# CZY-Code/PHNet

Hardware: AMD Instinct MI355X
Metric: clips/s (5x3x320x800) fwd+bwd (higher is better)
Workload: dtype f32 storage / accumulation, every product as an EXACT three-term bf16 split (6 bf16 MFMAs, f32-MFMA accuracy); 1 GPU; 5-frame clip 3x320x800, resnet34 + router + lane head, fwd+bwd+AdamW, 1 clip/GPU/step, random-init weights; parallelism=dp1, launch=hipGraph replay of the whole step

## Files before the change

### phnet_amd/csrc/assign.hip

```cpp
#include "assign_device.h"

namespace {

using namespace phassign;

__global__ __launch_bounds__(4 * NT) void lane_assign_kernel(
    const float* __restrict__ pred, const float* __restrict__ tgt, int N, int L, int S, float img_w, float img_h,
    int64_t* __restrict__ rows_by_col, int64_t* __restrict__ rows_sorted, int32_t* __restrict__ n_valid_out,
    float* __restrict__ cost_out)
{
    extern __shared__ float cost[];
    lane_assign_block<false, 4>(pred, tgt, N, L, S, img_w, img_h, rows_by_col, rows_sorted, n_valid_out, cost_out, cost);
}

__global__ __launch_bounds__(4 * NT) void lane_assign_tokens_kernel(
    const float* __restrict__ pred, const float* __restrict__ tgt, int N, int L, int S, float img_w, float img_h,
    int64_t* __restrict__ rows_by_col, int64_t* __restrict__ rows_sorted, const float* __restrict__ feat, int E,
    float* __restrict__ tokens, unsigned char* __restrict__ valid)
{
    extern __shared__ float cost[];
    float* part = cost + N * MAXL;
    const int e = threadIdx.x % E, grp = threadIdx.x / E, groups = (4 * NT) / E;
    float s = 0.f;
    if (grp < groups)
        for (int n = grp; n < N; n += groups) s += feat[(size_t)n * E + e];
    lane_assign_block<false, 4>(pred, tgt, N, L, S, img_w, img_h, rows_by_col, rows_sorted, nullptr, nullptr, cost);
    if (grp < groups) part[grp * E + e] = s;
    __syncthreads();
    if (grp != 0) return;
    float total = 0.f;
    for (int g2 = 0; g2 < groups; ++g2) total += part[g2 * E + e];
    float possum = 0.f;
    int cnt = 0;
    for (int l = 0; l < L; ++l) {
        const long long r = rows_sorted[l];
        const bool ok = r >= 0 && r < N;
        const float v = ok ? feat[(size_t)r * E + e] : 0.f;
        tokens[(size_t)l * E + e] = v;
        possum += v;
        cnt += ok;
        if (e == 0) valid[l] = ok;
    }
    tokens[(size_t)L * E + e] = (total - possum) / (float)(N - cnt);
    if (e == 0) valid[L] = 1;
}

__global__ __launch_bounds__(4 * NT) void lane_assign_many_kernel(
    const float* __restrict__ pred, const float* __restrict__ tgt, int N, int L, int S, float img_w, float img_h,
    int64_t* __restrict__ rows, int64_t* __restrict__ cols, int32_t* __restrict__ n_pairs)
{
    extern __shared__ float cost[];
    lane_assign_block<true, 4>(pred, tgt, N, L, S, img_w, img_h, nullptr, nullptr, nullptr, nullptr, cost, 0.5f, rows, cols, n_pairs);
}

}
PHNET_API int phnet_lane_assign(const float* pred, const float* tgt, int32_t N, int32_t L, int32_t S,
                                float img_w, float img_h, int64_t* rows_by_col, int64_t* rows_sorted,
                                int32_t* n_valid, float* cost, void* stream)
{
    if (N < 1 || N > NT || L < 0 || L > MAXL || S < 1 || S > 250) return PHNET_ERR_ARG;
    if (L == 0) return PHNET_OK;
    if (!pred || !tgt || !rows_by_col || !rows_sorted) return PHNET_ERR_ARG;
    hipLaunchKernelGGL(lane_assign_kernel, dim3(1), dim3(4 * NT), (size_t)N * MAXL * sizeof(float), (hipStream_t)stream,
                       pred, tgt, N, L, S, img_w, img_h, rows_by_col, rows_sorted, n_valid, cost);
    return phnet_launch_status();
}

PHNET_API int phnet_lane_assign_one2many(const float* pred, const float* tgt, int32_t N, int32_t L, int32_t S,
                                         float img_w, float img_h, int64_t* rows, int64_t* cols, int32_t* n_pairs, void* stream)
{
    if (N < 1 || N > NT || L < 1 || L > MAXL || S < 1 || S > 250) return PHNET_ERR_ARG;
    if (!pred || !tgt || !rows || !cols) return PHNET_ERR_ARG;
    hipLaunchKernelGGL(lane_assign_many_kernel, dim3(1), dim3(4 * NT), (size_t)2 * N * MAXL * sizeof(float), (hipStream_t)stream,
                       pred, tgt, N, L, S, img_w, img_h, rows, cols, n_pairs);
    return phnet_launch_status();
}

PHNET_API int phnet_lane_assign_tokens(const float* pred, const float* tgt, int32_t N, int32_t L, int32_t S, float img_w, float img_h,
                                       int64_t* rows_by_col, int64_t* rows_sorted, const float* feat, int32_t E,
                                       float* tokens, uint8_t* valid, void* stream)
{
    if (N < 1 || N > NT || L < 1 || L > MAXL || S < 1 || S > 250 || E < 1 || E > 256 || (4 * NT) % E) return PHNET_ERR_ARG;
    if (!pred || !tgt || !rows_by_col || !rows_sorted || !feat || !tokens || !valid) return PHNET_ERR_ARG;
    const size_t lds = ((size_t)N * MAXL + (size_t)4 * NT) * sizeof(float);
    hipLaunchKernelGGL(lane_assign_tokens_kernel, dim3(1), dim3(4 * NT), lds, (hipStream_t)stream,
                       pred, tgt, N, L, S, img_w, img_h, rows_by_col, rows_sorted, feat, E, tokens, valid);
    return phnet_launch_status();
}
```

### phnet_amd/csrc/assign_device.h

```cpp
#pragma once
#include "common.h"

namespace phassign {

constexpr int NT = 256;
constexpr int MAXL = 4;

template <int WAVES = 4>
__device__ __forceinline__ float block_max(float v, float* red) {
    v = wave_max(v);
    __syncthreads();
    if ((threadIdx.x & 63) == 0) red[threadIdx.x >> 6] = v;
    __syncthreads();
    float m = red[0];
#pragma unroll
    for (int i = 1; i < WAVES; ++i) m = fmaxf(m, red[i]);
    return m;
}

template <bool MANY = false, int QUAD = 1>
__device__ __forceinline__ void lane_assign_block(
    const float* __restrict__ pred, const float* __restrict__ tgt, int N, int L, int S, float img_w, float img_h,
    int64_t* __restrict__ rows_by_col, int64_t* __restrict__ rows_sorted, int32_t* __restrict__ n_valid_out,
    float* __restrict__ cost_out, float* cost ,
    float focal_alpha = 0.25f, int64_t* __restrict__ many_rows = nullptr, int64_t* __restrict__ many_cols = nullptr,
    int32_t* __restrict__ many_n = nullptr)
{
    __shared__ float t_x[MAXL][256];
    __shared__ float t_len[MAXL], red[4 * QUAD];
    __shared__ int t_valid[MAXL], top_rows[MAXL][MAXL], best_combo;
    __shared__ float combo_cost[NT];
    __shared__ unsigned char gone[NT];
    __shared__ int ks[MAXL], comp[MAXL], many_count, more;
    const int tid = threadIdx.x;
    const int W = 6 + S;
    if (tid < NT) gone[tid] = 0;

    if (tid < MAXL) {
        t_valid[tid] = (tid < L) && (tgt[tid * W + 1] == 1.0f);
        t_len[tid] = 0.f;
    }
    for (int i = tid; i < L * S; i += NT * QUAD) t_x[i / S][i % S] = tgt[(i / S) * W + 6 + (i % S)];
    __syncthreads();
    if (tid < L) {
        int n = 0;
        for (int k = 0; k < S; ++k) { const float t = t_x[tid][k]; n += !((t < 0.f) || (t >= img_w)); }
        t_len[tid] = (float)n;
    }
    __syncthreads();

    if constexpr (QUAD == 4) {
        const int a = tid & (NT - 1), jq = tid / NT;
        const bool arow = a < N, on = arow && jq < L && t_valid[jq];
        const float* p = pred + (size_t)(arow ? a : 0) * W;
        float cls = 0.f, dist = 0.f, start = 0.f, theta = 0.f, iou = 0.f;
        float mx_d = -INFINITY, mx_s = -INFINITY, mx_t = -INFINITY;
        if (arow) {
            const float pr = 1.0f / (1.0f + expf(-p[1]));
            const float negc = -logf(1.0f - pr + 1e-12f) * (1.0f - focal_alpha) * (pr * pr);
            const float posc = -logf(pr + 1e-12f) * focal_alpha * ((1.0f - pr) * (1.0f - pr));
            cls = posc - negc;
        }
        if (on) {
            float d = 0.f, ovr = 0.f, uni = 0.f;
            const float* tx = t_x[jq];
            auto term = [&](int k, float xr) {
                const float x = xr * (img_w - 1.0f), t = tx[k];
                const bool ok = !(t < 0.f) && !(t >= img_w);
                d += ok ? fabsf(t - x) : 0.f;
                ovr += ok ? fminf(x + 15.f, t + 15.f) - fmaxf(x - 15.f, t - 15.f) : 0.f;
                uni += ok ? fmaxf(x + 15.f, t + 15.f) - fminf(x - 15.f, t - 15.f) : 0.f;
            };
            int k = 0;
            if ((W & 1) == 0) {
                for (; k + 1 < S; k += 16) {
                    float2 buf[8];
#pragma unroll
                    for (int u = 0; u < 8; ++u) {
                        const int kk = k + 2 * u;
                        buf[u] = *reinterpret_cast<const float2*>(p + 6 + (kk + 1 < S ? kk : 0));
                    }
#pragma unroll
                    for (int u = 0; u < 8; ++u) {
                        const int kk = k + 2 * u;
                        if (kk + 1 < S) { term(kk, buf[u].x); term(kk + 1, buf[u].y); }
                    }
                }
                k = S & ~1;
            }
            for (; k < S; ++k) term(k, p[6 + k]);
            dist = d / (t_len[jq] + 1e-9f);
            iou = ovr / (uni + 1e-9f);
            const float* tr = tgt + (size_t)jq * W;
            const float dy = p[2] * (img_h - 1.0f) - tr[2] * (img_h - 1.0f), dx = p[3] * (img_w - 1.0f) - tr[3] * (img_w - 1.0f);
            start = sqrtf(dy * dy + dx * dx);
            theta = fabsf(p[4] - tr[4]) * 180.f;
            mx_d = dist; mx_s = start; mx_t = theta;
        }
        mx_d = block_max<16>(mx_d, red);
        mx_s = block_max<16>(mx_s, red);
        mx_t = block_max<16>(mx_t, red);
        if (arow) {
            float c = INFINITY;
            if (on) {
                const float a_ = 1.0f - dist / (mx_d + 1e-4f);
                const float b_ = 1.0f - start / (mx_s + 1e-4f);
                const float t_ = 1.0f - theta / (mx_t + 1e-4f);
                const float prod = a_ * b_ * t_;
                c = -(prod * prod) * 3.0f + cls - iou;
            }
            cost[a * MAXL + jq] = c;
            if (MANY) cost[(N + a) * MAXL + jq] = on ? fmaxf(iou, 0.f) : -1.f;
            if (cost_out && jq < L) cost_out[(size_t)a * L + jq] = c;
        }
    } else {
    float dist[MAXL], start[MAXL], theta[MAXL], iou[MAXL], cls = 0.f;
    float mx_d = -INFINITY, mx_s = -INFINITY, mx_t = -INFINITY;
    const bool arow = tid < N;
    if (arow) {
        const float* p = pred + (size_t)tid * W;
        const float pr = 1.0f / (1.0f + expf(-p[1]));
        const float negc = -logf(1.0f - pr + 1e-12f) * (1.0f - focal_alpha) * (pr * pr);
        const float posc = -logf(pr + 1e-12f) * focal_alpha * ((1.0f - pr) * (1.0f - pr));
        cls = posc - negc;
        const float psy = p[2] * (img_h - 1.0f), psx = p[3] * (img_w - 1.0f), pth = p[4];
        float d[MAXL], ovr[MAXL], uni[MAXL];
#pragma unroll
        for (int j = 0; j < MAXL; ++j) d[j] = ovr[j] = uni[j] = 0.f;
        bool col_on[MAXL];
#pragma unroll
        for (int j = 0; j < MAXL; ++j) col_on[j] = j < L && t_valid[j];
        auto term = [&](int k, float xr) {
            const float x = xr * (img_w - 1.0f);
#pragma unroll
            for (int j = 0; j < MAXL; ++j) {
                const float t = t_x[j][k];
                const bool ok = col_on[j] && !(t < 0.f) && !(t >= img_w);
                d[j] += ok ? fabsf(t - x) : 0.f;
                ovr[j] += ok ? fminf(x + 15.f, t + 15.f) - fmaxf(x - 15.f, t - 15.f) : 0.f;
                uni[j] += ok ? fmaxf(x + 15.f, t + 15.f) - fminf(x - 15.f, t - 15.f) : 0.f;
            }
        };
        int k = 0;
        if ((W & 1) == 0)
            for (; k + 1 < S; k += 16) {
                float2 buf[8];
#pragma unroll
                for (int u = 0; u < 8; ++u) {
                    const int kk = k + 2 * u;
                    buf[u] = *reinterpret_cast<const float2*>(p + 6 + (kk + 1 < S ? kk : 0));
                }
#pragma unroll
                for (int u = 0; u < 8; ++u) {
                    const int kk = k + 2 * u;
                    if (kk + 1 < S) { term(kk, buf[u].x); term(kk + 1, buf[u].y); }
                }
            }
        k = ((W & 1) == 0) ? (S & ~1) : 0;
        for (; k < S; ++k) term(k, p[6 + k]);
#pragma unroll
        for (int j = 0; j < MAXL; ++j) {
            dist[j] = start[j] = theta[j] = iou[j] = 0.f;
            if (j >= L || !t_valid[j]) continue;
            dist[j] = d[j] / (t_len[j] + 1e-9f);
            iou[j] = ovr[j] / (uni[j] + 1e-9f);
            const float* tr = tgt + (size_t)j * W;
            const float dy = psy - tr[2] * (img_h - 1.0f), dx = psx - tr[3] * (img_w - 1.0f);
            start[j] = sqrtf(dy * dy + dx * dx);
            theta[j] = fabsf(pth - tr[4]) * 180.f;
            mx_d = fmaxf(mx_d, dist[j]); mx_s = fmaxf(mx_s, start[j]); mx_t = fmaxf(mx_t, theta[j]);
        }
    }
    mx_d = block_max(mx_d, red);
    mx_s = block_max(mx_s, red);
    mx_t = block_max(mx_t, red);
    if (arow) {
#pragma unroll
        for (int j = 0; j < MAXL; ++j) {
            float c = INFINITY;
            if (j < L && t_valid[j]) {
                const float a = 1.0f - dist[j] / (mx_d + 1e-4f);
                const float b = 1.0f - start[j] / (mx_s + 1e-4f);
                const float t = 1.0f - theta[j] / (mx_t + 1e-4f);
                const float prod = a * b * t;
                c = -(prod * prod) * 3.0f + cls - iou[j];
            }
            cost[tid * MAXL + j] = c;
            if (MANY) cost[(N + tid) * MAXL + j] = (j < L && t_valid[j]) ? fmaxf(iou[j], 0.f) : -1.f;
            if (cost_out && j < L) cost_out[(size_t)tid * L + j] = c;
        }
    }
    }
    __syncthreads();

    if (MANY) {
        const int j = tid >> 6, lane = tid & 63;
        if (j < MAXL) {
            const bool valid = j < L && t_valid[j];
            float sum = 0.f;
            int taken[MAXL];
            for (int r = 0; r < MAXL; ++r) {
                float bv = -INFINITY; int bi = 0x7fffffff;
                if (valid)
                    for (int i = lane; i < N; i += 64) {
                        bool tk = false;
                        for (int q = 0; q < r; ++q) tk |= (taken[q] == i);
                        const float v = cost[(N + i) * MAXL + j];
                        if (!tk && (v > bv || (v == bv && i < bi))) { bv = v; bi = i; }
                    }
#pragma unroll
                for (int off = 32; off > 0; off >>= 1) {
                    const float ov = __shfl_xor(bv, off, 64);
                    const int oi = __shfl_xor(bi, off, 64);
                    if (ov > bv || (ov == bv && oi < bi)) { bv = ov; bi = oi; }
                }
                taken[r] = bi;
                if (valid && bi != 0x7fffffff) sum += bv;
            }
            if (lane == 0) {
                const int k = (int)sum;
                ks[j] = valid ? (k < 1 ? 1 : k) : 0;
            }
        }
        if (tid == 0) many_count = 0;
        __syncthreads();
        if (tid == 0) {
            int c = 0;
            for (int j = 0; j < MAXL; ++j) { comp[j] = c; c += (j < L && t_valid[j]); }
            int kc[MAXL] = {0, 0, 0, 0};
            for (int j = 0; j < MAXL; ++j) if (j < L && t_valid[j]) kc[comp[j]] = ks[j];
            for (int j = 0; j < MAXL; ++j) ks[j] = kc[j];
            more = (kc[0] + kc[1] + kc[2] + kc[3]) > 0;
        }
        __syncthreads();
    }
    for (int round = 0; round < (MANY ? MAXL + 1 : 1); ++round) {
    if (MANY && !more) break;
    {
        const int j = tid >> 6, lane = tid & 63;
        if (j < MAXL) {
            const bool valid = j < L && t_valid[j];
            for (int r = 0; r < MAXL; ++r) {
                float bv = INFINITY; int bi = 0x7fffffff;
                if (valid)
                    for (int i = lane; i < N; i += 64) {
                        bool taken = gone[i] != 0;
                        for (int q = 0; q < r; ++q) taken |= (top_rows[j][q] == i);
                        const float c = cost[i * MAXL + j];
                        if (!taken && (c < bv || (c == bv && i < bi))) { bv = c; bi = i; }
                    }
#pragma unroll
                for (int off = 32; off > 0; off >>= 1) {
                    const float ov = __shfl_xor(bv, off, 64);
                    const int oi = __shfl_xor(bi, off, 64);
                    if (ov < bv || (ov == bv && oi < bi)) { bv = ov; bi = oi; }
                }
                if (lane == 0) top_rows[j][r] = valid ? bi : -1;
                __builtin_amdgcn_wave_barrier();
            }
        }
    }
    __syncthreads();

    {
        int rows[MAXL];
        float total = 0.f;
        bool ok = true;
#pragma unroll
        for (int j = 0; j < MAXL; ++j) {
            const int pick = (tid >> (2 * j)) & 3;
            const bool valid = j < L && t_valid[j];
            rows[j] = valid ? top_rows[j][pick] : -1;
            if (!valid) { ok = ok && pick == 0; continue; }
            if (rows[j] < 0 || rows[j] == 0x7fffffff) { ok = false; continue; }
            total += cost[rows[j] * MAXL + j];
#pragma unroll
            for (int q = 0; q < j; ++q) ok = ok && !(rows[q] >= 0 && rows[q] == rows[j]);
        }
        if (tid < NT) combo_cost[tid] = ok ? total : INFINITY;
    }
    __syncthreads();
    if (tid < 64) {
        float bv = INFINITY; int bi = 0x7fffffff;
        for (int c = tid; c < NT; c += 64) {
            const float v = combo_cost[c];
            if (v < bv || (v == bv && c < bi)) { bv = v; bi = c; }
        }
#pragma unroll
        for (int off = 32; off > 0; off >>= 1) {
            const float ov = __shfl_xor(bv, off, 64);
            const int oi = __shfl_xor(bi, off, 64);
            if (ov < bv || (ov == bv && oi < bi)) { bv = ov; bi = oi; }
        }
        if (tid == 0) best_combo = bi;
    }
    __syncthreads();
    if (tid == 0) {
        int rows[MAXL], nv = 0;
        for (int j = 0; j < MAXL; ++j) {
            const bool valid = j < L && t_valid[j];
            rows[j] = (valid && best_combo != 0x7fffffff) ? top_rows[j][(best_combo >> (2 * j)) & 3] : -1;
            if (j < L && rows_by_col) rows_by_col[j] = rows[j];
            nv += rows[j] >= 0;
        }
        for (int a = 0; a < MAXL; ++a)
            for (int b = a + 1; b < MAXL; ++b) {
                const bool swap = (rows[b] >= 0) && (rows[a] < 0 || rows[b] < rows[a]);
                if (swap) { const int t = rows[a]; rows[a] = rows[b]; rows[b] = t; }
            }
        if (!MANY) {
            for (int j = 0; j < L; ++j) rows_sorted[j] = rows[j];
            if (n_valid_out) *n_valid_out = nv;
        } else {
            int lab[MAXL];
            for (int p_ = 0; p_ < MAXL; ++p_) {
                lab[p_] = -1;
                if (rows[p_] < 0) continue;
                for (int j = 0; j < MAXL; ++j)
                    if (j < L && t_valid[j] && best_combo != 0x7fffffff && top_rows[j][(best_combo >> (2 * j)) & 3] == rows[p_]) lab[p_] = j;
            }
            for (int p_ = 0; p_ < MAXL; ++p_) {
                if (rows[p_] < 0 || ks[p_] <= 0) continue;
                many_rows[many_count] = rows[p_];
                many_cols[many_count] = lab[p_];
                ++many_count;
                gone[rows[p_]] = 1;
            }
            int any = 0;
            for (int j = 0; j < MAXL; ++j) { if (ks[j] > 0) --ks[j]; any += ks[j]; }
            more = any > 0 && nv > 0;
        }
    }
    __syncthreads();
    }
    if (MANY && tid == 0) {
        for (int i = many_count; i < MAXL * MAXL; ++i) { many_rows[i] = -1; many_cols[i] = -1; }
        if (many_n) *many_n = many_count;
    }
}


}
```

### phnet_amd/libs/models/Router4OL.py

```python
import copy
import math

import torch
import torch.nn as nn

from phnet_amd import functional as PF
from phnet_amd.arena import SinkPool, grad_sink
from phnet_amd.trunk import encoder_forward
from ..ops import nms
from ..utils.lane import Lane
from .fpn import FPN
from .resnet import ResNetWrapper
from .Router import AdaptiveRouter4Lane
from .utils.dynamic_head import DynamicConv
from .utils.transformer import TransformerDecoder, TransformerDecoderLayer


def LinearModule(hidden_dim):
    return nn.ModuleList([nn.Linear(hidden_dim, hidden_dim), nn.ReLU(inplace=False)])


class PositionalEncodingLearned(nn.Module):
    def __init__(self, num_embeddings, num_pos_feats=256):
        super().__init__()
# ... 193 lines not shown
        if self.training:
            self.priors, self.priors_on_featmap = self.generate_priors_from_embeddings()
        parts = {k: v.split(1, dim=0) for k, v in self.stage0_front(fmaps0).items()}
        return [{k: parts[k][t] for k in parts} for t in range(fmaps0.shape[0])]

    def forward(self, x, last_cuts=None, stage0=None):
        levels = list(x)[::-1]
        last_cuts = last_cuts or []
        if self.training and stage0 is None:
            self.priors, self.priors_on_featmap = self.generate_priors_from_embeddings()
        priors, on_map = self.priors.unsqueeze(0), self.priors_on_featmap.unsqueeze(0)
        pro_feat = self.pro_embedding.weight.unsqueeze(0)
        out_a, out_b, attn_feats, gates = [], [], [], []
        for stage in range(self.refine_layers):
            mem = None
            if len(last_cuts):
                mem = (torch.cat([fr[stage][0] for fr in last_cuts], dim=0), torch.cat([fr[stage][1] for fr in last_cuts], dim=0))
            if stage == 0 and stage0 is not None:
                r = self.stage_back(stage0, 0, priors, mem)
            else:
                r = self.stage_forward(levels[stage], stage, priors, on_map, pro_feat, mem)
            pro_feat = r["local"].detach()
            out_a.append(r["pred_a"]); out_b.append(r["pred_b"]); attn_feats.append(r["attn"]); gates.append(r["gate"])
            if stage != self.refine_layers - 1:
                from phnet_amd import hip_ops as K
                priors, on_map = K.blend_priors(r["gate"].detach().contiguous(), r["lines_a"].detach().contiguous(),
                                                r["lines_b"].detach().contiguous(), self.sample_x_indexs)
        return {"predictions_fir": out_a, "predictions_sec": out_b}, attn_feats, gates

    def forward_clips(self, x, last_cuts=None, stage0=None, stream=None):
        levels = list(x)[::-1]
        last_cuts = last_cuts or []
        B, N = levels[0].shape[0], self.num_priors
        priors = self.priors.unsqueeze(0).expand(B, -1, -1)
        on_map = self.priors_on_featmap.unsqueeze(0).expand(B, -1, -1).contiguous()
        pro_feat = self.pro_embedding.weight.unsqueeze(0).expand(B, -1, -1)
        pos = self.PositionEmbedding.embed.weight.unsqueeze(0).expand(B, -1, -1)
        out_a, out_b, attn_feats, gates = [], [], [], []
        from phnet_amd import hip_ops as K
        for stage in range(self.refine_layers):
            front = stage0 if (stage == 0 and stage0 is not None) else self.stage_front(levels[stage], stage, priors, on_map, pro_feat)
            local = front["local"]
            attn = torch.cat([local, pos], dim=-1) if stream is None else torch.cat([local, pos], dim=-1, out=stream.feat[stage])
            if stream is not None:
                mem, valid = stream.window[stage], stream.window_valid[stage]
                feat = self.transformer_Dec(tgt=attn.reshape(B * N, -1), memory=mem.reshape(-1, mem.shape[-1]),
                                            memory_key_valid=valid.reshape(-1), batch=B)
                feat = K.stream_select(attn, stream.has_memory, feat.reshape(B, N, -1))
            elif len(last_cuts):
                mem = torch.cat([fr[stage][0] for fr in last_cuts], dim=1)
                valid = torch.cat([fr[stage][1] for fr in last_cuts], dim=1)
                feat = self.transformer_Dec(tgt=attn.reshape(B * N, -1), memory=mem.reshape(-1, mem.shape[-1]),
                                            memory_key_valid=valid.reshape(-1), batch=B)
            else:
                feat = attn
            pred_b, lines_b = self._branch(feat.reshape(B, N, -1), priors, True)
            pro_feat = local.detach()
            out_a.append(front["pred_a"]); out_b.append(pred_b); attn_feats.append(attn); gates.append(front["gate"])
            if stage != self.refine_layers - 1:
                priors, on_map = K.blend_priors(front["gate"].detach().contiguous(), front["lines_a"].detach().contiguous(),
                                                lines_b.detach().contiguous(), self.sample_x_indexs)
        return {"predictions_fir": out_a, "predictions_sec": out_b}, attn_feats, gates

    def predictions_to_pred(self, predictions, ori_img_h=None, cut_height=0):
        rows = predictions.detach().cpu()
        ys_all = self.prior_ys.detach().cpu().double()
        lanes = []
        for row in rows:
            xs = row[6:].clone()
            start = min(max(0, int(round(row[2].item() * self.n_strips))), self.n_strips)
            end = min(start + int(round(row[5].item())) - 1, self.n_offsets - 1)
            inside = ((xs[:start] >= 0.) & (xs[:start] <= 1.)).numpy()
            outside = ~(inside[::-1].cumprod()[::-1].astype(bool))
            xs[end + 1:] = -2
            xs[:start][torch.from_numpy(outside.copy())] = -2
            sel = xs >= 0
            lx, ly = xs[sel].flip(0).double(), ys_all[sel].flip(0)
            if lx.numel() <= 1:
                continue
            lanes.append(Lane(points=torch.stack([lx, ly], dim=1).numpy(),
                              metadata={"start_x": row[3], "start_y": row[2], "conf": row[1]}))
        return lanes

    def decode_device(self, lines: torch.Tensor):
        from phnet_amd import hip_ops as K
        tp = self.cfg.test_parameters
        return K.lane_decode(lines.contiguous(), tp.conf_threshold, tp.nms_thres, self.cfg.max_lanes, self.img_w)

    def blended_lines(self, outputs, gates):
        d = torch.stack(gates, dim=0).mean(dim=0)
        return outputs["predictions_sec"][-1] * d + outputs["predictions_fir"][-1] * (1 - d)

    def decode_frame(self, outputs, gates):
        return self.decode_device(self.blended_lines(outputs, gates))

    def points_device(self, dec, out=None):
        from phnet_amd import hip_ops as K
        return K.lane_points(dec["kept_rows"].contiguous(), dec["num"].contiguous(), self.prior_ys.contiguous(), out=out)

    def get_lanes(self, output, org_size=None, crop_size=0, as_lanes=True):
        decoded, keep_inds, keep = [], None, []
        for predictions in output:
            scores = torch.softmax(predictions[:, :2], dim=1)[:, 1]
            keep_inds = scores >= self.cfg.test_parameters.conf_threshold
            cand = predictions[keep_inds]
            keep = []
            if cand.shape[0] == 0:
                decoded.append([])
                continue
            rows = torch.cat([cand[:, :4], cand[:, 5:]], dim=-1).detach().clone()
            rows[:, 3] = rows[:, 3] * (self.img_w - 1)
            rows[:, 4] = rows[:, 4] * self.n_strips
            rows[:, 5:] = rows[:, 5:] * (self.img_w - 1)
            keep, num_to_keep, _ = nms(rows.contiguous(), scores[keep_inds].contiguous(),
                                       overlap=self.cfg.test_parameters.nms_thres, top_k=self.cfg.max_lanes)
            keep = keep[:int(num_to_keep)]
            kept = cand[keep].clone()
            if kept.shape[0] == 0:
                decoded.append([])
                continue
            kept[:, 5] = torch.round(kept[:, 5] * self.n_strips)
            decoded.append(self.predictions_to_pred(kept) if as_lanes else kept)
        return decoded, keep_inds, keep


def _points_of(det, kept_rows: torch.Tensor, nums: torch.Tensor) -> dict:
    lead = tuple(nums.shape)
    out = det.points_device({"kept_rows": kept_rows.reshape(-1, *kept_rows.shape[-2:]), "num": nums.reshape(-1)})
    return {k: v.view(*lead, *v.shape[1:]) for k, v in out.items()}


class DeviceResults:
    stream_class = "LaneStream"

    def lanes_from_device(self, kept_rows: torch.Tensor, nums: torch.Tensor):
        rows, n = kept_rows.cpu(), nums.cpu().tolist()
        return {"lane_lines": [self.head.predictions_to_pred(rows[t, :n[t]]) if n[t] else [] for t in range(len(n))]}

    def infer_points_device(self, frames: torch.Tensor):
        rows, nums, anchors = (self.infer_device(frames) if frames.dim() == 4 else self.infer_clips_device(frames))[:3]
        return rows, nums, anchors, _points_of(self.head, rows, nums)

    def polylines_from_device(self, polylines: dict, kept_rows: torch.Tensor):
        from phnet_amd import polylines as P
        return P.to_host(polylines["points"], polylines["count"], polylines["lanes_num"], polylines["slot"], kept_rows)

    def open_stream(self, streams: int = 1, frame_hw=None, graph: bool = True, reset_every=None, raw=None, polylines: bool = False,
                    track: bool = False, max_tracks=None, max_age=None, match_thres=None, render=None):
        from phnet_amd import stream
        return getattr(stream, self.stream_class)(self, streams=streams, frame_hw=frame_hw, graph=graph, reset_every=reset_every,
                                                  raw=raw, polylines=polylines, track=track, max_tracks=max_tracks, max_age=max_age,
                                                  match_thres=match_thres, render=render)

    def track_clips(self, kept_rows: torch.Tensor, nums: torch.Tensor, max_tracks=None, max_age=None, match_thres=None):
        from phnet_amd import hip_ops as K
        from phnet_amd.tracking import TrackState, track_defaults
        M, age, thr = track_defaults(self, max_tracks, max_age, match_thres)
        one = nums.dim() == 1
        rows, n = (kept_rows[None], nums[None]) if one else (kept_rows, nums)
        state = TrackState(rows.shape[0], M, rows.shape[-1] - 6, rows.device)
        out = K.lane_track(rows.contiguous(), n.contiguous(), state, thr, age)
        return (out["track_id"][0], out["hits"][0]) if one else (out["track_id"], out["hits"])


BRANCH_B_SITES = 1 << 10


class _Stacked(list):
    stacked = None


class _BranchBDeferred(torch.autograd.Function):

    @staticmethod
    def forward(ctx, model, pre_pred, pri_all, rings, valids, n_tok, pri0, *rest):
        ctx.model, ctx.rings, ctx.valids, ctx.n_tok = model, rings, valids, n_tok
        ctx.params = rest[n_tok:]
        ctx.save_for_backward(pri_all, *[t.detach() for t in rest[:n_tok]])
        return pre_pred.view_as(pre_pred)

    @staticmethod
    def backward(ctx, d_pred):
        pri_all, *tokens = ctx.saved_tensors
        det = ctx.model.detNet
        S, T = len(tokens), tokens[0].shape[0]
        need_pri = ctx.needs_input_grad[6]
        wanted = [i for i, p in enumerate(ctx.params) if ctx.needs_input_grad[7 + ctx.n_tok + i]]
        outer_cache, det._branch_cache = det._branch_cache, None
        try:
            with torch.enable_grad():
                tok = torch.cat(tokens, dim=0).requires_grad_()
                pri = pri_all.detach().requires_grad_(need_pri)
                pred = ctx.model._branch_b_batch(tok, pri, ctx.rings, ctx.valids, S, T)
                grads = torch.autograd.grad([pred], [tok] + ([pri] if need_pri else []) + [ctx.params[i] for i in wanted],
                                            [d_pred.contiguous()], allow_unused=True)
        finally:
            det._branch_cache = outer_cache
        ctx.rings = ctx.valids = None
        d_tok = grads[0].split(T, dim=0)
        d_pri0 = grads[1][:T] if need_pri else None
        d_par = [None] * len(ctx.params)
        for j, i in enumerate(wanted):
            d_par[i] = grads[1 + int(need_pri) + j]
        return (None, None, None, None, None, None, d_pri0) + tuple(d_tok) + tuple(d_par)


class RouterOL(nn.Module, DeviceResults):
    SCHEDULES = ("stage", "frame")

    def __init__(self, cfg, criterion=None):
        super().__init__()
        self.backbone = Encoder(cfg=cfg)
        self.detNet = DetNetV2(cfg=cfg)
        self.criterion = criterion
        self.save_freq_max = cfg.save_freq_max
        self.crop_size = cfg.dscfg.crop_size
        self.org_size = (cfg.dscfg.org_height, cfg.dscfg.org_width)
        self.sync_free_eval = True
        self.batch_stage0 = True
        self.schedule = "stage"
        self.defer_branch_b = True

    @property
    def head(self):
        return self.detNet

    @property
    def schedule(self) -> str:
        return self._schedule

    @schedule.setter
    def schedule(self, name: str):
        if name not in self.SCHEDULES:
            raise ValueError(f"RouterOL.schedule: one of {self.SCHEDULES} expected, got {name!r}")
        self._schedule = name

    def _begin_clip(self):
        det = self.detNet
        det._branch_cache = None
        det._sink_pool = SinkPool() if self.training else None
        for head in det.DHead_series:
            head.begin_clip(det._sink_pool)
        if det.priors.grad_fn is not None:
            det.priors = det.priors.detach()
            det.priors_on_featmap = det.priors_on_featmap.detach()

    def infer_device(self, frame: torch.Tensor):
        self._begin_clip()
        feats = self.backbone(frame)
        last_cuts, rows, nums, anchors = [], [], [], []
        stage0 = self.detNet.stage0_all_frames(feats[-1]) if self.batch_stage0 else None
        for t in range(frame.shape[0]):
            cur = tuple(f[t:t + 1] for f in feats)
            outputs, cur_cut, gates = self.detNet(cur, last_cuts, None if stage0 is None else stage0[t])
            dec = self.detNet.decode_device(self.detNet.blended_lines(outputs, gates)[0])
            rows.append(dec["kept_rows"]); nums.append(dec["num"]); anchors.append(dec["anchors"])
            last_cuts.append([self._tokens(feat.detach(), dec["anchors_sorted"]) for feat in cur_cut])
            if t >= self.save_freq_max:
                last_cuts.pop(0)
        self._begin_clip()
        return torch.stack(rows), torch.stack(nums), torch.stack(anchors)

    def infer_clips_device(self, frames: torch.Tensor):
        from phnet_amd import hip_ops as K
        B, T = frames.shape[:2]
        self._begin_clip()
        feats = self.backbone(frames.transpose(0, 1).reshape(T * B, *frames.shape[2:]))
        det = self.detNet
        front0 = det.stage0_front(feats[-1])
        last_cuts, rows, nums, anchors = [], [], [], []
        for t in range(T):
            cur = tuple(f[t * B:(t + 1) * B] for f in feats)
            outputs, cur_cut, gates = det.forward_clips(cur, last_cuts, {k: v[t * B:(t + 1) * B] for k, v in front0.items()})
            dec = det.decode_frame(outputs, gates)
            rows.append(dec["kept_rows"]); nums.append(dec["num"]); anchors.append(dec["anchors"])
            last_cuts.append([K.memory_tokens(feat.detach().contiguous(), dec["anchors_sorted"].contiguous()) for feat in cur_cut])
            if t >= self.save_freq_max:
                last_cuts.pop(0)
        self._begin_clip()
        return torch.stack(rows, dim=1), torch.stack(nums, dim=1), torch.stack(anchors, dim=1)

    def forward_clips_train(self, frames: torch.Tensor, lanes: torch.Tensor):
        from phnet_amd import hip_ops as K
        B, T = frames.shape[:2]
        self._begin_clip()
        PF.DropoutStream.begin_step(frames.device)
        feats = self.backbone(frames.transpose(0, 1).reshape(T * B, *frames.shape[2:]))
        det = self.detNet
        det.priors, det.priors_on_featmap = det.generate_priors_from_embeddings()
        front0 = {k: v.split(B, dim=0) for k, v in det.stage0_front(feats[-1]).items()}
        levels = [f.split(B, dim=0) for f in feats]
        last_cuts, total_loss = [], 0.0
        for t in range(T):
            cur = tuple(lv[t] for lv in levels)
            outputs, cur_cut, gates = det.forward_clips(cur, last_cuts, {k: v[t] for k, v in front0.items()})
            matched_all = []
            per_clip = {k: [p.split(1, dim=0) for p in v] for k, v in outputs.items()}
            gate_clip = [gt.split(1, dim=0) for gt in gates]
            for b in range(B):
                out_b = {k: [ps[b] for ps in v] for k, v in per_clip.items()}
                matched, loss_b = self.criterion(out_b, lanes[b, t:t + 1], [gs[b] for gs in gate_clip])
                total_loss = total_loss + loss_b
                matched_all.append(matched)
            with torch.no_grad():
                tokens = []
                for s_i, feat in enumerate(cur_cut):
                    rows = torch.stack([matched_all[b][s_i] for b in range(B)])
                    tokens.append(K.memory_tokens(feat.detach().contiguous(), rows))
                last_cuts.append(tokens)
                if t >= self.save_freq_max:
                    last_cuts.pop(0)
        self._begin_clip()
        return total_loss

    def _branch_b_batch(self, tok, pri, rings, valids, S: int, T: int):
        det = self.detNet
        N, E, W = det.num_priors, tok.shape[-1], self.save_freq_max
        feat = tok
        if T > 1:
            L1 = rings[0].shape[1]
            tokv = tok.view(S, T, N, E)
            tgt = tokv[:, 1:].reshape(S * (T - 1) * N, E)
            ring = getattr(rings, "stacked", None)
            valid = getattr(valids, "stacked", None)
            if ring is None or valid is None or ring.shape[0] != S:
                ring = torch.stack(rings) if S > 1 else rings[0].unsqueeze(0)
                valid = torch.stack(valids) if S > 1 else valids[0].unsqueeze(0)
            st = ring.stride()
            mem = ring.as_strided((S, T - 1, W * L1, E), (st[0], st[1], E, 1), ring.storage_offset() + st[1]).reshape(-1, E)
            sv = valid.stride()
            key_valid = valid.as_strided((S, T - 1, W * L1), (sv[0], sv[1], 1), valid.storage_offset() + sv[1]).reshape(-1)
            with PF.DropoutStream.items(BRANCH_B_SITES, 0, N):
                dec = det.transformer_Dec(tgt=tgt, memory=mem, memory_key_valid=key_valid, batch=S * (T - 1))
            feat = torch.cat([tokv[:, :1], dec.view(S, T - 1, N, E)], dim=1).reshape(S * T, N, E)
        pred, _ = det._branch(feat, pri, True)
        return pred

    def _clip_loss(self, per_frame, lanes):
        outs = [{"predictions_fir": fr["predictions_fir"], "predictions_sec": fr["predictions_sec"]} for fr in per_frame]
        if hasattr(self.criterion, "clip_loss"):
            return self.criterion.clip_loss(outs, lanes, [fr["gates"] for fr in per_frame])
        total_loss = 0.0
        for t, out in enumerate(outs):
            _, frame_loss = self.criterion(out, lanes[t:t + 1], per_frame[t]["gates"])
            total_loss = total_loss + frame_loss
        return total_loss

    def train_clip_stage_major(self, frame: torch.Tensor, lanes: torch.Tensor):
        from phnet_amd import hip_ops as K
        det = self.detNet
        T, S, N = frame.shape[0], det.refine_layers, det.num_priors
        W, L1 = self.save_freq_max, lanes.shape[1] + 1
        dev = frame.device
        feats = self.backbone(frame)
        levels = list(feats)[::-1]
        det.priors, det.priors_on_featmap = det.generate_priors_from_embeddings()
        priors = det.priors.unsqueeze(0).expand(T, -1, -1)
        on_map = det.priors_on_featmap.unsqueeze(0).expand(T, -1, -1).contiguous()
        pro = det.pro_embedding.weight.unsqueeze(0).expand(T, -1, -1)
        E = 2 * det.fc_hidden_dim
        defer = self.defer_branch_b
        det._branch_weights(True)
        per_frame = [{"predictions_fir": [], "predictions_sec": [], "gates": []} for _ in range(T)]
        pos = det.PositionEmbedding.embed.weight.unsqueeze(0).expand(T, -1, -1)
        tokens, rings, valids, pre_pred, pri_used = [], _Stacked(), _Stacked(), [], []
        pri0 = priors
        rings.stacked = torch.zeros((S, W + T, L1, E), dtype=torch.float32, device=dev)
        valids.stacked = torch.zeros((S, W + T, L1), dtype=torch.bool, device=dev)
        for stage in range(S):
            front = det.stage_front(levels[stage], stage, priors, on_map, pro)
            attn_all = torch.cat([front["local"], pos], dim=-1)
            ring, ring_valid = rings.stacked[stage], valids.stacked[stage]
            if defer:
                src, pri_src = attn_all.detach(), priors.detach()
            else:
                src = attn_all
                pri_src = priors
            tok_t = src.split(1, dim=0)
            pri_t = pri_src.split(1, dim=0) if pri_src.requires_grad else [pri_src[t:t + 1] for t in range(T)]
            lines_b, preds_b = [], []
            for t in range(T):
                mem = (ring[t:t + W].view(-1, 1, E), ring_valid[t:t + W].view(-1)) if t > 0 else None
                with torch.set_grad_enabled(not defer), PF.DropoutStream.items(BRANCH_B_SITES, stage * (T - 1) + t - 1 if t else 0, 0):
                    pred_b, line_b = det.forward_second(mem, tok_t[t].transpose(0, 1), stage, pri_t[t])
                with torch.no_grad():
                    K.lane_assign_tokens(pred_b[0].detach().contiguous(), lanes[t].contiguous(), det.img_w, det.img_h,
                                         tok_t[t].detach().contiguous(), (ring[W + t], ring_valid[W + t]))
                preds_b.append(pred_b)
                lines_b.append(line_b.detach())
            pa = front["pred_a"].split(1, dim=0)
            gt = front["gate"].split(1, dim=0)
            for t in range(T):
                per_frame[t]["predictions_fir"].append(pa[t])
                per_frame[t]["gates"].append(gt[t])
                if not defer:
                    per_frame[t]["predictions_sec"].append(preds_b[t])
            if defer:
                tokens.append(attn_all); rings.append(ring); valids.append(ring_valid)
                pre_pred.append(torch.cat(preds_b, dim=0)); pri_used.append(pri_src)
            if stage != S - 1:
                priors, on_map = K.blend_priors(front["gate"].detach().contiguous(), front["lines_a"].detach().contiguous(),
                                                torch.cat(lines_b, dim=0), det.sample_x_indexs)
                pro = front["local"].detach()
        if defer:
            params = list(det.transformer_Dec.parameters())
            for name in ("cls_modules_sec", "reg_modules_sec", "iou_modules_sec", "cls_layers_sec", "reg_layers_sec", "iou_layers_sec"):
                params += list(getattr(det, name).parameters())
            pred_all = _BranchBDeferred.apply(self, torch.cat(pre_pred, dim=0), torch.cat(pri_used, dim=0), rings, valids, len(tokens),
                                              pri0, *tokens, *params)
            pb = pred_all.split(1, dim=0)
            for s_ in range(S):
                for t in range(T):
                    per_frame[t]["predictions_sec"].append(pb[s_ * T + t])
        return self._clip_loss(per_frame, lanes)

    def forward(self, inputs: dict):
        frame, lanes = inputs.values()
        if not frame.is_cuda:
            raise RuntimeError("phnet_amd runs on the GPU only: move the model and the clip to cuda")
        if frame.dim() == 5:
            if self.training:
                return self.forward_clips_train(frame, lanes)
            rows, nums, _ = self.infer_clips_device(frame)
            B = frame.shape[0]
            return [self.lanes_from_device(rows[b], nums[b]) for b in range(B)]
        if not self.training and self.sync_free_eval:
            rows, nums, _ = self.infer_device(frame)
            return self.lanes_from_device(rows, nums)
        T = frame.shape[0]
        self._begin_clip()
        if self.training:
            PF.DropoutStream.begin_step(frame.device)
            if self.schedule == "stage" and self.batch_stage0:
                loss = self.train_clip_stage_major(frame, lanes)
                self._begin_clip()
                return loss
        feats = self.backbone(frame)
        last_cuts = []
        total_loss = 0.0
        clip_outputs = {"lane_lines": []}
        per_level = [f.split(1, dim=0) for f in feats]
        stage0 = self.detNet.stage0_all_frames(feats[-1]) if self.batch_stage0 else None
        for t in range(T):
            cur = tuple(lv[t] for lv in per_level)
            outputs, cur_cut, gates = self.detNet(cur, last_cuts, None if stage0 is None else stage0[t])
            if self.training:
                matched, frame_loss = self.criterion(outputs, lanes[t:t + 1], gates)
                total_loss = total_loss + frame_loss
            else:
                lines = self.detNet.blended_lines(outputs, gates)
                lane_lines, keep_inds, keep = self.detNet.get_lanes(lines, self.org_size, self.crop_size)
                clip_outputs["lane_lines"].append(lane_lines[0])
            with torch.no_grad():
                if self.training:
                    last_cuts.append(self.saveMemory(matched, cur_cut))
                else:
                    last_cuts.append(self.saveMemory4Test(keep_inds, keep, cur_cut))
                if t >= self.save_freq_max:
                    last_cuts.pop(0)
        self._begin_clip()
        return total_loss if self.training else clip_outputs

    def _tokens(self, feat, rows):
        from phnet_amd import hip_ops as K
        return K.memory_tokens(feat.contiguous(), rows.contiguous())

    def saveMemory(self, matched_indices, curr_cut):
        return [self._tokens(feat.detach(), rows) for rows, feat in zip(matched_indices, curr_cut)]

    def saveMemory4Test(self, keep_inds, keep, curr_cut):
        rows = torch.full((self.detNet.cfg.max_lanes,), -1, dtype=torch.int64, device=curr_cut[0].device)
        if len(keep):
            idx = torch.sort(torch.where(keep_inds)[0][keep])[0]
            rows[: idx.numel()] = idx
        return [self._tokens(feat.detach(), rows) for feat in curr_cut]
```

Measured before the change: 65.28 clips/s.

## Skip last-frame token assignment and streamline lane-assign kernel reductions and prefetch

The Python side stops computing memory tokens and lane assignments for the final frame of each clip, because nothing consumes them afterwards. The HIP lane-assign kernel now prefetches prediction x-coordinates into registers before the target staging barrier. It computes target lengths with wave ballots, caches target heads in LDS and fuses the three block max reductions into one. Candidate selection keeps costs in registers and uses a DPP arg-min/arg-max in place of shuffle loops. The token kernel also overlaps the feature sum loads with assignment and reads sorted rows from LDS, at the cost of more register pressure and more complex code.

```diff
diff --git a/phnet_amd/csrc/assign.hip b/phnet_amd/csrc/assign.hip
--- a/phnet_amd/csrc/assign.hip
+++ b/phnet_amd/csrc/assign.hip
@@ -19,23 +19,41 @@
     float* __restrict__ tokens, unsigned char* __restrict__ valid)
 {
     extern __shared__ float cost[];
+    __shared__ int sorted[MAXL];
     float* part = cost + N * MAXL;
+    constexpr int CB = 32;
     const int e = threadIdx.x % E, grp = threadIdx.x / E, groups = (4 * NT) / E;
+    const int mine = (grp < groups && grp < N) ? (N - grp + groups - 1) / groups : 0;
+    const int head = mine > CB ? mine - CB : 0;
     float s = 0.f;
-    if (grp < groups)
-        for (int n = grp; n < N; n += groups) s += feat[(size_t)n * E + e];
-    lane_assign_block<false, 4>(pred, tgt, N, L, S, img_w, img_h, rows_by_col, rows_sorted, nullptr, nullptr, cost);
+    for (int i = 0; i < head; ++i) s += feat[(size_t)(grp + i * groups) * E + e];
+    float fb[CB];
+#pragma unroll
+    for (int u = 0; u < CB; ++u) fb[u] = feat[(size_t)(head + u < mine ? grp + (head + u) * groups : 0) * E + e];
+    lane_assign_block<false, 4, 18>(pred, tgt, N, L, S, img_w, img_h, rows_by_col, rows_sorted, nullptr, nullptr, cost, 0.25f, nullptr,
+                                    nullptr, nullptr, sorted);
+#pragma unroll
+    for (int u = 0; u < CB; ++u) s = head + u < mine ? s + fb[u] : s;
     if (grp < groups) part[grp * E + e] = s;
     __syncthreads();
     if (grp != 0) return;
+    bool oks[MAXL];
+    float vs[MAXL];
+#pragma unroll
+    for (int l = 0; l < MAXL; ++l) {
+        const int r = l < L ? sorted[l] : -1;
+        oks[l] = r >= 0 && r < N;
+        vs[l] = feat[(size_t)(oks[l] ? r : 0) * E + e];
+    }
     float total = 0.f;
     for (int g2 = 0; g2 < groups; ++g2) total += part[g2 * E + e];
     float possum = 0.f;
     int cnt = 0;
-    for (int l = 0; l < L; ++l) {
-        const long long r = rows_sorted[l];
-        const bool ok = r >= 0 && r < N;
-        const float v = ok ? feat[(size_t)r * E + e] : 0.f;
+#pragma unroll
+    for (int l = 0; l < MAXL; ++l) {
+        if (l >= L) break;
+        const bool ok = oks[l];
+        const float v = ok ? vs[l] : 0.f;
         tokens[(size_t)l * E + e] = v;
         possum += v;
         cnt += ok;
diff --git a/phnet_amd/csrc/assign_device.h b/phnet_amd/csrc/assign_device.h
--- a/phnet_amd/csrc/assign_device.h
+++ b/phnet_amd/csrc/assign_device.h
@@ -5,29 +5,65 @@
 
 constexpr int NT = 256;
 constexpr int MAXL = 4;
-
-template <int WAVES = 4>
-__device__ __forceinline__ float block_max(float v, float* red) {
-    v = wave_max(v);
-    __syncthreads();
-    if ((threadIdx.x & 63) == 0) red[threadIdx.x >> 6] = v;
-    __syncthreads();
-    float m = red[0];
-#pragma unroll
-    for (int i = 1; i < WAVES; ++i) m = fmaxf(m, red[i]);
-    return m;
-}
-
-template <bool MANY = false, int QUAD = 1>
+constexpr int CAND = NT / 64;
+
+template <int V> struct PfTag { static constexpr int value = V; };
+
+template <int WAVES>
+__device__ __forceinline__ void block_max3(float& a, float& b, float& c, float (*red)[3]) {
+    a = wave_max(a); b = wave_max(b); c = wave_max(c);
+    if ((threadIdx.x & 63) == 0) {
+        float* r = red[threadIdx.x >> 6];
+        r[0] = a; r[1] = b; r[2] = c;
+    }
+    __syncthreads();
+    a = red[0][0]; b = red[0][1]; c = red[0][2];
+#pragma unroll
+    for (int i = 1; i < WAVES; ++i) { a = fmaxf(a, red[i][0]); b = fmaxf(b, red[i][1]); c = fmaxf(c, red[i][2]); }
+}
+
+__device__ __forceinline__ float wave_len(const float* tx, int S, float img_w) {
+    const int lane = threadIdx.x & 63;
+    int n = 0;
+    for (int k0 = 0; k0 < S; k0 += 64) {
+        const int k = k0 + lane;
+        const float t = tx[k];
+        n += __popcll(__ballot(k < S && !((t < 0.f) || (t >= img_w))));
+    }
+    return (float)n;
+}
+
+template <int CTRL, bool LESS>
+__device__ __forceinline__ void arg_best_step(float& bv, int& bi) {
+    const float ov = dpp_move<CTRL>(bv);
+    const int oi = __builtin_amdgcn_update_dpp(bi, bi, CTRL, 0xf, 0xf, false);
+    const bool take = LESS ? (ov < bv || (ov == bv && oi < bi)) : (ov > bv || (ov == bv && oi < bi));
+    bv = take ? ov : bv;
+    bi = take ? oi : bi;
+}
+template <bool LESS>
+__device__ __forceinline__ void wave_arg_best(float& bv, int& bi) {
+    arg_best_step<0xb1, LESS>(bv, bi);
+    arg_best_step<0x4e, LESS>(bv, bi);
+    arg_best_step<0x124, LESS>(bv, bi);
+    arg_best_step<0x128, LESS>(bv, bi);
+    arg_best_step<0x142, LESS>(bv, bi);
+    arg_best_step<0x143, LESS>(bv, bi);
+    bv = __builtin_bit_cast(float, __builtin_amdgcn_readlane(__builtin_bit_cast(int, bv), 63));
+    bi = __builtin_amdgcn_readlane(bi, 63);
+}
+
+template <bool MANY = false, int QUAD = 1, int MAXPF = 36>
 __device__ __forceinline__ void lane_assign_block(
     const float* __restrict__ pred, const float* __restrict__ tgt, int N, int L, int S, float img_w, float img_h,
     int64_t* __restrict__ rows_by_col, int64_t* __restrict__ rows_sorted, int32_t* __restrict__ n_valid_out,
     float* __restrict__ cost_out, float* cost ,
     float focal_alpha = 0.25f, int64_t* __restrict__ many_rows = nullptr, int64_t* __restrict__ many_cols = nullptr,
-    int32_t* __restrict__ many_n = nullptr)
+    int32_t* __restrict__ many_n = nullptr, int* sorted_lds = nullptr)
 {
     __shared__ float t_x[MAXL][256];
-    __shared__ float t_len[MAXL], red[4 * QUAD];
+    __shared__ float t_hd[MAXL][3];
+    __shared__ float red[4 * QUAD][3];
     __shared__ int t_valid[MAXL], top_rows[MAXL][MAXL], best_combo;
     __shared__ float combo_cost[NT];
     __shared__ unsigned char gone[NT];
@@ -36,27 +72,35 @@
     const int W = 6 + S;
     if (tid < NT) gone[tid] = 0;
 
-    if (tid < MAXL) {
-        t_valid[tid] = (tid < L) && (tgt[tid * W + 1] == 1.0f);
-        t_len[tid] = 0.f;
-    }
-    for (int i = tid; i < L * S; i += NT * QUAD) t_x[i / S][i % S] = tgt[(i / S) * W + 6 + (i % S)];
-    __syncthreads();
-    if (tid < L) {
-        int n = 0;
-        for (int k = 0; k < S; ++k) { const float t = t_x[tid][k]; n += !((t < 0.f) || (t >= img_w)); }
-        t_len[tid] = (float)n;
-    }
-    __syncthreads();
-
+    auto stage = [&]() {
+        if (tid < MAXL) t_valid[tid] = (tid < L) && (tgt[tid * W + 1] == 1.0f);
+        for (int i = tid; i < L * S; i += NT * QUAD) t_x[i / S][i % S] = tgt[(i / S) * W + 6 + (i % S)];
+        if (tid >= 64 && tid < 64 + 3 * MAXL) {
+            const int j = (tid - 64) / 3, c = (tid - 64) % 3;
+            if (j < L) t_hd[j][c] = tgt[j * W + 2 + c];
+        }
+        __syncthreads();
+    };
+
+    auto cost_phase = [&](auto pf) {
+    constexpr int PF = decltype(pf)::value;
     if constexpr (QUAD == 4) {
         const int a = tid & (NT - 1), jq = tid / NT;
-        const bool arow = a < N, on = arow && jq < L && t_valid[jq];
+        const bool arow = a < N;
         const float* p = pred + (size_t)(arow ? a : 0) * W;
+        const float p1 = p[1], p2 = p[2], p3 = p[3], p4 = p[4];
+        float2 xb[PF > 0 ? PF : 1];
+        if constexpr (PF > 0) {
+#pragma unroll
+            for (int u = 0; u < PF; ++u) xb[u] = *reinterpret_cast<const float2*>(p + 6 + (2 * u + 1 < S ? 2 * u : 0));
+        }
+        stage();
+        const bool lab = jq < L && t_valid[jq], on = arow && lab;
+        const float tl = lab ? wave_len(t_x[jq], S, img_w) : 0.f;
         float cls = 0.f, dist = 0.f, start = 0.f, theta = 0.f, iou = 0.f;
         float mx_d = -INFINITY, mx_s = -INFINITY, mx_t = -INFINITY;
         if (arow) {
-            const float pr = 1.0f / (1.0f + expf(-p[1]));
+            const float pr = 1.0f / (1.0f + expf(-p1));
             const float negc = -logf(1.0f - pr + 1e-12f) * (1.0f - focal_alpha) * (pr * pr);
             const float posc = -logf(pr + 1e-12f) * focal_alpha * ((1.0f - pr) * (1.0f - pr));
             cls = posc - negc;
@@ -71,35 +115,39 @@
                 ovr += ok ? fminf(x + 15.f, t + 15.f) - fmaxf(x - 15.f, t - 15.f) : 0.f;
                 uni += ok ? fmaxf(x + 15.f, t + 15.f) - fminf(x - 15.f, t - 15.f) : 0.f;
             };
-            int k = 0;
-            if ((W & 1) == 0) {
-                for (; k + 1 < S; k += 16) {
-                    float2 buf[8];
-#pragma unroll
-                    for (int u = 0; u < 8; ++u) {
-                        const int kk = k + 2 * u;
-                        buf[u] = *reinterpret_cast<const float2*>(p + 6 + (kk + 1 < S ? kk : 0));
+            if constexpr (PF > 0) {
+#pragma unroll
+                for (int u = 0; u < PF; ++u)
+                    if (2 * u + 1 < S) { term(2 * u, xb[u].x); term(2 * u + 1, xb[u].y); }
+            } else {
+                int k = 0;
+                if ((W & 1) == 0) {
+                    for (; k + 1 < S; k += 16) {
+                        float2 buf[8];
+#pragma unroll
+                        for (int u = 0; u < 8; ++u) {
+                            const int kk = k + 2 * u;
+                            buf[u] = *reinterpret_cast<const float2*>(p + 6 + (kk + 1 < S ? kk : 0));
+                        }
+#pragma unroll
+                        for (int u = 0; u < 8; ++u) {
+                            const int kk = k + 2 * u;
+                            if (kk + 1 < S) { term(kk, buf[u].x); term(kk + 1, buf[u].y); }
+                        }
                     }
-#pragma unroll
-                    for (int u = 0; u < 8; ++u) {
-                        const int kk = k + 2 * u;
-                        if (kk + 1 < S) { term(kk, buf[u].x); term(kk + 1, buf[u].y); }
-                    }
+                    k = S & ~1;
                 }
-                k = S & ~1;
-            }
-            for (; k < S; ++k) term(k, p[6 + k]);
-            dist = d / (t_len[jq] + 1e-9f);
+                for (; k < S; ++k) term(k, p[6 + k]);
+            }
+            dist = d / (tl + 1e-9f);
             iou = ovr / (uni + 1e-9f);
-            const float* tr = tgt + (size_t)jq * W;
-            const float dy = p[2] * (img_h - 1.0f) - tr[2] * (img_h - 1.0f), dx = p[3] * (img_w - 1.0f) - tr[3] * (img_w - 1.0f);
+            const float* tr = t_hd[jq];
+            const float dy = p2 * (img_h - 1.0f) - tr[0] * (img_h - 1.0f), dx = p3 * (img_w - 1.0f) - tr[1] * (img_w - 1.0f);
             start = sqrtf(dy * dy + dx * dx);
-            theta = fabsf(p[4] - tr[4]) * 180.f;
+            theta = fabsf(p4 - tr[2]) * 180.f;
             mx_d = dist; mx_s = start; mx_t = theta;
         }
-        mx_d = block_max<16>(mx_d, red);
-        mx_s = block_max<16>(mx_s, red);
-        mx_t = block_max<16>(mx_t, red);
+        block_max3<16>(mx_d, mx_s, mx_t, red);
         if (arow) {
             float c = INFINITY;
             if (on) {
@@ -117,13 +165,23 @@
     float dist[MAXL], start[MAXL], theta[MAXL], iou[MAXL], cls = 0.f;
     float mx_d = -INFINITY, mx_s = -INFINITY, mx_t = -INFINITY;
     const bool arow = tid < N;
+    const float* p = pred + (size_t)(arow ? tid : 0) * W;
+    const float p1 = p[1], p2 = p[2], p3 = p[3], p4 = p[4];
+    float2 xb[PF > 0 ? PF : 1];
+    if constexpr (PF > 0) {
+#pragma unroll
+        for (int u = 0; u < PF; ++u) xb[u] = *reinterpret_cast<const float2*>(p + 6 + (2 * u + 1 < S ? 2 * u : 0));
+    }
+    stage();
+    float tl[MAXL];
+#pragma unroll
+    for (int j = 0; j < MAXL; ++j) tl[j] = (j < L && t_valid[j]) ? wave_len(t_x[j], S, img_w) : 0.f;
     if (arow) {
-        const float* p = pred + (size_t)tid * W;
-        const float pr = 1.0f / (1.0f + expf(-p[1]));
+        const float pr = 1.0f / (1.0f + expf(-p1));
         const float negc = -logf(1.0f - pr + 1e-12f) * (1.0f - focal_alpha) * (pr * pr);
         const float posc = -logf(pr + 1e-12f) * focal_alpha * ((1.0f - pr) * (1.0f - pr));
         cls = posc - negc;
-        const float psy = p[2] * (img_h - 1.0f), psx = p[3] * (img_w - 1.0f), pth = p[4];
+        const float psy = p2 * (img_h - 1.0f), psx = p3 * (img_w - 1.0f), pth = p4;
         float d[MAXL], ovr[MAXL], uni[MAXL];
 #pragma unroll
         for (int j = 0; j < MAXL; ++j) d[j] = ovr[j] = uni[j] = 0.f;
@@ -141,39 +199,43 @@
                 uni[j] += ok ? fmaxf(x + 15.f, t + 15.f) - fminf(x - 15.f, t - 15.f) : 0.f;
             }
         };
-        int k = 0;
-        if ((W & 1) == 0)
-            for (; k + 1 < S; k += 16) {
-                float2 buf[8];
-#pragma unroll
-                for (int u = 0; u < 8; ++u) {
-                    const int kk = k + 2 * u;
-                    buf[u] = *reinterpret_cast<const float2*>(p + 6 + (kk + 1 < S ? kk : 0));
+        if constexpr (PF > 0) {
+#pragma unroll
+            for (int u = 0; u < PF; ++u)
+                if (2 * u + 1 < S) { term(2 * u, xb[u].x); term(2 * u + 1, xb[u].y); }
+        } else {
+            int k = 0;
+            if ((W & 1) == 0)
+                for (; k + 1 < S; k += 16) {
+                    float2 buf[8];
+#pragma unroll
+                    for (int u = 0; u < 8; ++u) {
+                        const int kk = k + 2 * u;
+                        buf[u] = *reinterpret_cast<const float2*>(p + 6 + (kk + 1 < S ? kk : 0));
+                    }
+#pragma unroll
+                    for (int u = 0; u < 8; ++u) {
+                        const int kk = k + 2 * u;
+                        if (kk + 1 < S) { term(kk, buf[u].x); term(kk + 1, buf[u].y); }
+                    }
                 }
-#pragma unroll
-                for (int u = 0; u < 8; ++u) {
-                    const int kk = k + 2 * u;
-                    if (kk + 1 < S) { term(kk, buf[u].x); term(kk + 1, buf[u].y); }
-                }
-            }
-        k = ((W & 1) == 0) ? (S & ~1) : 0;
-        for (; k < S; ++k) term(k, p[6 + k]);
+            k = ((W & 1) == 0) ? (S & ~1) : 0;
+            for (; k < S; ++k) term(k, p[6 + k]);
+        }
 #pragma unroll
         for (int j = 0; j < MAXL; ++j) {
             dist[j] = start[j] = theta[j] = iou[j] = 0.f;
             if (j >= L || !t_valid[j]) continue;
-            dist[j] = d[j] / (t_len[j] + 1e-9f);
+            dist[j] = d[j] / (tl[j] + 1e-9f);
             iou[j] = ovr[j] / (uni[j] + 1e-9f);
-            const float* tr = tgt + (size_t)j * W;
-            const float dy = psy - tr[2] * (img_h - 1.0f), dx = psx - tr[3] * (img_w - 1.0f);
+            const float* tr = t_hd[j];
+            const float dy = psy - tr[0] * (img_h - 1.0f), dx = psx - tr[1] * (img_w - 1.0f);
             start[j] = sqrtf(dy * dy + dx * dx);
-            theta[j] = fabsf(pth - tr[4]) * 180.f;
+            theta[j] = fabsf(pth - tr[2]) * 180.f;
             mx_d = fmaxf(mx_d, dist[j]); mx_s = fmaxf(mx_s, start[j]); mx_t = fmaxf(mx_t, theta[j]);
         }
     }
-    mx_d = block_max(mx_d, red);
-    mx_s = block_max(mx_s, red);
-    mx_t = block_max(mx_t, red);
+    block_max3<4>(mx_d, mx_s, mx_t, red);
     if (arow) {
 #pragma unroll
         for (int j = 0; j < MAXL; ++j) {
@@ -191,30 +253,35 @@
         }
     }
     }
+    };
+    if ((W & 1) == 0 && S <= 36) cost_phase(PfTag<18>{});
+    else if (MAXPF >= 36 && (W & 1) == 0 && S <= 72) cost_phase(PfTag<(MAXPF >= 36 ? 36 : 0)>{});
+    else cost_phase(PfTag<0>{});
     __syncthreads();
 
     if (MANY) {
         const int j = tid >> 6, lane = tid & 63;
         if (j < MAXL) {
             const bool valid = j < L && t_valid[j];
+            float cv[CAND]; bool ex[CAND];
+#pragma unroll
+            for (int q = 0; q < CAND; ++q) {
+                const int i = lane + 64 * q;
+                ex[q] = !valid || i >= N;
+                cv[q] = ex[q] ? 0.f : cost[(N + i) * MAXL + j];
+            }
             float sum = 0.f;
-            int taken[MAXL];
+#pragma unroll
             for (int r = 0; r < MAXL; ++r) {
                 float bv = -INFINITY; int bi = 0x7fffffff;
-                if (valid)
-                    for (int i = lane; i < N; i += 64) {
-                        bool tk = false;
-                        for (int q = 0; q < r; ++q) tk |= (taken[q] == i);
-                        const float v = cost[(N + i) * MAXL + j];
-                        if (!tk && (v > bv || (v == bv && i < bi))) { bv = v; bi = i; }
-                    }
-#pragma unroll
-                for (int off = 32; off > 0; off >>= 1) {
-                    const float ov = __shfl_xor(bv, off, 64);
-                    const int oi = __shfl_xor(bi, off, 64);
-                    if (ov > bv || (ov == bv && oi < bi)) { bv = ov; bi = oi; }
+#pragma unroll
+                for (int q = 0; q < CAND; ++q) {
+                    const int i = lane + 64 * q;
+                    if (!ex[q] && (cv[q] > bv || (cv[q] == bv && i < bi))) { bv = cv[q]; bi = i; }
                 }
-                taken[r] = bi;
+                wave_arg_best<false>(bv, bi);
+#pragma unroll
+                for (int q = 0; q < CAND; ++q) ex[q] = ex[q] || (bi == lane + 64 * q);
                 if (valid && bi != 0x7fffffff) sum += bv;
             }
             if (lane == 0) {
@@ -240,23 +307,25 @@
         const int j = tid >> 6, lane = tid & 63;
         if (j < MAXL) {
             const bool valid = j < L && t_valid[j];
+            float cv[CAND]; bool ex[CAND];
+#pragma unroll
+            for (int q = 0; q < CAND; ++q) {
+                const int i = lane + 64 * q;
+                ex[q] = !valid || i >= N || gone[i] != 0;
+                cv[q] = ex[q] ? 0.f : cost[i * MAXL + j];
+            }
+#pragma unroll
             for (int r = 0; r < MAXL; ++r) {
                 float bv = INFINITY; int bi = 0x7fffffff;
-                if (valid)
-                    for (int i = lane; i < N; i += 64) {
-                        bool taken = gone[i] != 0;
-                        for (int q = 0; q < r; ++q) taken |= (top_rows[j][q] == i);
-                        const float c = cost[i * MAXL + j];
-                        if (!taken && (c < bv || (c == bv && i < bi))) { bv = c; bi = i; }
-                    }
-#pragma unroll
-                for (int off = 32; off > 0; off >>= 1) {
-                    const float ov = __shfl_xor(bv, off, 64);
-                    const int oi = __shfl_xor(bi, off, 64);
-                    if (ov < bv || (ov == bv && oi < bi)) { bv = ov; bi = oi; }
+#pragma unroll
+                for (int q = 0; q < CAND; ++q) {
+                    const int i = lane + 64 * q;
+                    if (!ex[q] && (cv[q] < bv || (cv[q] == bv && i < bi))) { bv = cv[q]; bi = i; }
                 }
+                wave_arg_best<true>(bv, bi);
+#pragma unroll
+                for (int q = 0; q < CAND; ++q) ex[q] = ex[q] || (bi == lane + 64 * q);
                 if (lane == 0) top_rows[j][r] = valid ? bi : -1;
-                __builtin_amdgcn_wave_barrier();
             }
         }
     }
@@ -286,12 +355,7 @@
             const float v = combo_cost[c];
             if (v < bv || (v == bv && c < bi)) { bv = v; bi = c; }
         }
-#pragma unroll
-        for (int off = 32; off > 0; off >>= 1) {
-            const float ov = __shfl_xor(bv, off, 64);
-            const int oi = __shfl_xor(bi, off, 64);
-            if (ov < bv || (ov == bv && oi < bi)) { bv = ov; bi = oi; }
-        }
+        wave_arg_best<true>(bv, bi);
         if (tid == 0) best_combo = bi;
     }
     __syncthreads();
@@ -310,6 +374,8 @@
             }
         if (!MANY) {
             for (int j = 0; j < L; ++j) rows_sorted[j] = rows[j];
+            if (sorted_lds)
+                for (int j = 0; j < MAXL; ++j) sorted_lds[j] = rows[j];
             if (n_valid_out) *n_valid_out = nv;
         } else {
             int lab[MAXL];
diff --git a/phnet_amd/libs/models/Router4OL.py b/phnet_amd/libs/models/Router4OL.py
--- a/phnet_amd/libs/models/Router4OL.py
+++ b/phnet_amd/libs/models/Router4OL.py
@@ -519,6 +519,8 @@
                 matched, loss_b = self.criterion(out_b, lanes[b, t:t + 1], [gs[b] for gs in gate_clip])
                 total_loss = total_loss + loss_b
                 matched_all.append(matched)
+            if t == T - 1:
+                break
             with torch.no_grad():
                 tokens = []
                 for s_i, feat in enumerate(cur_cut):
@@ -600,11 +602,13 @@
                 mem = (ring[t:t + W].view(-1, 1, E), ring_valid[t:t + W].view(-1)) if t > 0 else None
                 with torch.set_grad_enabled(not defer), PF.DropoutStream.items(BRANCH_B_SITES, stage * (T - 1) + t - 1 if t else 0, 0):
                     pred_b, line_b = det.forward_second(mem, tok_t[t].transpose(0, 1), stage, pri_t[t])
+                preds_b.append(pred_b)
+                lines_b.append(line_b.detach())
+                if t == T - 1:
+                    continue
                 with torch.no_grad():
                     K.lane_assign_tokens(pred_b[0].detach().contiguous(), lanes[t].contiguous(), det.img_w, det.img_h,
                                          tok_t[t].detach().contiguous(), (ring[W + t], ring_valid[W + t]))
-                preds_b.append(pred_b)
-                lines_b.append(line_b.detach())
             pa = front["pred_a"].split(1, dim=0)
             gt = front["gate"].split(1, dim=0)
             for t in range(T):
```

After: 65.99 clips/s, median of 6. 1.01x the previous value.
